# jankammeth/BA-path-planning

Hardware: AMD Instinct MI355X
Metric: SCP iterations/sec (N agents x K waypoints) (higher is better)
Workload: dtype f64

## Files before the change

### ba-path-planning_amd/csrc/scp_common.h

```cpp
#pragma once
#include <hip/hip_runtime.h>

#include <cstdarg>
#include <cstdint>
#include <cstdio>
#include <cstring>

#include "scp_hip.h"

struct scp_stats_mirror {
  scp_pair_stats stats;
  unsigned long long n_spec;
  double pts[6];
  double rel[64];
  volatile unsigned long long seq;
};

constexpr int SCP_SMALL_MAX_WG = 2048;

struct scp_ctx {
  int device;
  int n_cu;
  hipStream_t stream;
  char err[512];
  double* d_scratch;
  double* h_scratch;
  double* h_scratch_dev;
  hipEvent_t ev0, ev1;
  hipEvent_t pair_ev0, pair_ev1;
  bool pair_timed;
  bool pair_ran;
  bool last_pass_small;
  double* tm_scratch;
  size_t tm_bytes;
  uint32_t* cmp_map;
  size_t cmp_map_bytes;
  uint32_t* cmp_tot;
  size_t cmp_tot_bytes;
  scp_stats_mirror* h_mirror;
  scp_stats_mirror* d_mirror;
  unsigned long long mirror_seq;
  unsigned long long* wg_part;
  uint32_t* wg_rows;
  size_t wg_rows_bytes;
  unsigned* d_ticket;
  int timing;
  int small_pass;
  unsigned long long rel_seq;
  void* gen_ws;
  size_t gen_ws_bytes;
  void* sep_ws;
  size_t sep_ws_bytes;
  unsigned long long* sep_n_solved;
  int* h_gen_flag;
  int* d_gen_flag;
};

static inline int scp_fail(scp_ctx* ctx, int code, const char* fmt, ...) {
  if (ctx) {
    va_list ap;
    va_start(ap, fmt);
    vsnprintf(ctx->err, sizeof(ctx->err), fmt, ap);
    va_end(ap);
  }
  return code;
}

#define SCP_HIP_CHECK(ctx, call)                                                                     \
  do {                                                                                               \
    hipError_t e_ = (call);                                                                          \
    if (e_ != hipSuccess)                                                                            \
      return scp_fail((ctx), SCP_ERR_HIP, "%s failed: %s (%s:%d)", #call, hipGetErrorString(e_),    \
                      __FILE__, __LINE__);                                                           \
  } while (0)

#define SCP_REQUIRE(ctx, cond, ...)                                   \
  do {                                                                \
    if (!(cond)) return scp_fail((ctx), SCP_ERR_INVALID, __VA_ARGS__); \
  } while (0)

static inline int64_t scp_pairs(int N) { return (int64_t)N * (N - 1) / 2; }
static inline int scp_cdiv(int64_t a, int64_t b) { return (int)((a + b - 1) / b); }

hipError_t scp_raise_lds_limit(int device, const void* kernel, size_t bytes);

bool scp_wait_host_word(volatile unsigned long long* word, unsigned long long seq, int timeout_s);

int scp_check_pair_range(scp_ctx* ctx, int N, int K, int D, int64_t q_begin, int64_t q_end);

int scp_ctx_wait_stats(scp_ctx* ctx, scp_pair_stats* out);

int scp_violations_from_solution(scp_ctx* ctx, int N, int K, int D, double R, double h, int64_t q_begin, int64_t q_end,
                                 const double* pos_prev, const double* x_tm, const double* p0, const double* v0, double* x_out,
                                 double* pos_out, double feas_tol, int64_t* new_rows, int64_t new_cap, uint32_t* sel_bitmap,
                                 scp_pair_stats* stats, const double* rel_prev ,
                                 int64_t* spec_rows , int64_t spec_cap,
                                 uint32_t* spec_bitmap, double spec_margin, bool* fused);
void scp_ctx_mirror_rel(scp_ctx* ctx, int64_t n, double* out);
int scp_select_from_solution(scp_ctx* ctx, int N, int K, int D, double R, double h, int64_t q_begin, int64_t q_end,
                             const double* x_tm, const double* p0, const double* v0, double* x_out, double* pos_out,
                             double margin, int64_t* sel_rows, int64_t sel_cap, uint32_t* sel_bitmap, scp_pair_stats* stats,
                             bool* fused);
int scp_launch_kinematics_copy(scp_ctx* ctx, int N, int K, int D, double h, const double* acc, const double* p0,
                               const double* v0, double* pos_out, double* vel_out, double* acc_copy);
const double* scp_qp_solution_tm(const scp_qp* qp);

int scp_qp_reset_add_rows_at(scp_qp* qp, const double* x0, int64_t n, const int64_t* rows, const double* pos_prev,
                             const double* p0, const double* v0, double R);
int scp_qp_add_rows_from_pass(scp_qp* qp, int64_t n, const int64_t* rows, const double* eta, const double* l_col,
                              int64_t q_begin, int64_t q_end);

int scp_launch_add_rows_at(scp_ctx* ctx, int N, int K, int D, int64_t base, int64_t n, const int64_t* rows,
                           const double* pos_prev, const double* p0, const double* v0, double R, double h, const double* Qx,
                           int64_t* w_row, int* wk, int* wi, int* wj, double* weta, double* wl, double* zc, double* yc);

int scp_launch_gemm(scp_ctx* ctx, int use_mfma, int R, int M, int C, double alpha, const double* A,
                    const double* X, double beta, double* Y);
int scp_launch_to_time_major(scp_ctx* ctx, int N, int K, int D, const double* src, double* dst);
int scp_launch_from_time_major(scp_ctx* ctx, int N, int K, int D, const double* src, double* dst);
int scp_launch_bounds_time_major(scp_ctx* ctx, int N, int K, int D, double h, const double* limits_host,
                                 const double* space_host, const double* p0, const double* v0,
                                 const double* pf, const double* vf, double* l_tm, double* u_tm,
                                 double* states_out );
```

### ba-path-planning_amd/csrc/scp_kernels.hip

```cpp
#include "scp_common.h"
#include "scp_pair_device.h"

#include <sys/prctl.h>
#include <time.h>

#include <atomic>
#include <chrono>
#include <cmath>
#include <cstdlib>
#include <map>
#include <mutex>
#include <type_traits>
#include <utility>

extern "C" int scp_abi_version(void) { return SCP_ABI_VERSION; }

extern "C" int scp_ctx_create(int device, void* hip_stream, scp_ctx** out) {
  if (!out) return SCP_ERR_INVALID;
  *out = nullptr;
  if (hipSetDevice(device) != hipSuccess) return SCP_ERR_HIP;
  scp_ctx* ctx = new scp_ctx();
  memset(ctx, 0, sizeof(*ctx));
  ctx->device = device;
  ctx->stream = (hipStream_t)hip_stream;
  ctx->timing = 1;
  ctx->small_pass = getenv("SCP_NO_SMALL_PASS") ? 0 : 1;
  if (hipDeviceGetAttribute(&ctx->n_cu, hipDeviceAttributeMultiprocessorCount, device) != hipSuccess) ctx->n_cu = 0;
  if (hipMalloc(&ctx->d_scratch, 72 * sizeof(double)) != hipSuccess ||
      hipMemset(ctx->d_scratch, 0, 72 * sizeof(double)) != hipSuccess ||
      hipHostMalloc(&ctx->h_scratch, 72 * sizeof(double)) != hipSuccess ||
      memset(ctx->h_scratch, 0, 72 * sizeof(double)) == nullptr ||
      hipHostGetDevicePointer((void**)&ctx->h_scratch_dev, ctx->h_scratch, 0) != hipSuccess ||
      hipHostMalloc(&ctx->h_mirror, sizeof(scp_stats_mirror)) != hipSuccess ||
      hipHostGetDevicePointer((void**)&ctx->d_mirror, ctx->h_mirror, 0) != hipSuccess ||
      hipEventCreate(&ctx->ev0) != hipSuccess || hipEventCreate(&ctx->ev1) != hipSuccess ||
      hipEventCreate(&ctx->pair_ev0) != hipSuccess || hipEventCreate(&ctx->pair_ev1) != hipSuccess ||
      hipMalloc(&ctx->wg_part, 4 * SCP_SMALL_MAX_WG * sizeof(unsigned long long)) != hipSuccess ||
      hipMalloc(&ctx->d_ticket, 64) != hipSuccess || hipMemset(ctx->d_ticket, 0, 64) != hipSuccess) {
    delete ctx;
    return SCP_ERR_HIP;
  }
  *out = ctx;
  return SCP_OK;
}

extern "C" int scp_ctx_set_option(scp_ctx* ctx, const char* key, int value) {
  if (!ctx || !key) return SCP_ERR_INVALID;
  if (strcmp(key, "kernel_timing") == 0) {
    ctx->timing = value ? 1 : 0;
    if (!ctx->timing) ctx->pair_timed = false;
    return SCP_OK;
  }
  if (strcmp(key, "single_launch_passes") == 0) {
    ctx->small_pass = value ? 1 : 0;
    return SCP_OK;
  }
  return scp_fail(ctx, SCP_ERR_INVALID, "ctx_set_option: unknown key '%s'", key);
}

extern "C" void scp_ctx_destroy(scp_ctx* ctx) {
  if (!ctx) return;
  (void)hipSetDevice(ctx->device);
  (void)hipStreamSynchronize(ctx->stream);
  (void)hipFree(ctx->d_scratch);
  if (ctx->wg_part) (void)hipFree(ctx->wg_part);
  if (ctx->wg_rows) (void)hipFree(ctx->wg_rows);
  if (ctx->d_ticket) (void)hipFree(ctx->d_ticket);
  if (ctx->cmp_map) (void)hipFree(ctx->cmp_map);
  if (ctx->cmp_tot) (void)hipFree(ctx->cmp_tot);
  if (ctx->tm_scratch) (void)hipFree(ctx->tm_scratch);
  if (ctx->gen_ws) (void)hipFree(ctx->gen_ws);
  if (ctx->sep_ws) (void)hipFree(ctx->sep_ws);
  if (ctx->h_gen_flag) (void)hipHostFree(ctx->h_gen_flag);
  (void)hipHostFree(ctx->h_scratch);
  (void)hipHostFree(ctx->h_mirror);
  (void)hipEventDestroy(ctx->ev0);
  (void)hipEventDestroy(ctx->ev1);
  (void)hipEventDestroy(ctx->pair_ev0);
  (void)hipEventDestroy(ctx->pair_ev1);
  delete ctx;
}

hipError_t scp_raise_lds_limit(int device, const void* kernel, size_t bytes) {
  static std::mutex mu;
  static std::map<std::pair<int, const void*>, size_t> allowed;
  std::lock_guard<std::mutex> lock(mu);
  size_t& have = allowed[std::make_pair(device, kernel)];
  if (have >= bytes) return hipSuccess;
  const hipError_t e = hipFuncSetAttribute(kernel, hipFuncAttributeMaxDynamicSharedMemorySize, (int)bytes);
  if (e == hipSuccess) have = bytes;
  return e;
}

static std::atomic<int> g_host_wait_mode{0};

extern "C" void scp_set_host_wait(int mode) {
  g_host_wait_mode.store(mode == 1 || mode == 2 ? mode : 0, std::memory_order_relaxed);
}

bool scp_wait_host_word(volatile unsigned long long* word, unsigned long long seq, int timeout_s) {
  const auto t0 = std::chrono::steady_clock::now();
  const int wait_mode = g_host_wait_mode.load(std::memory_order_relaxed);
  const bool sleepy = wait_mode != 0;
  const unsigned spin_first = wait_mode == 2 ? 0u : 2000u;
  if (sleepy) {
    static thread_local bool slack_set = false;
    if (!slack_set) {
      (void)prctl(PR_SET_TIMERSLACK, 1000UL, 0UL, 0UL, 0UL);
      slack_set = true;
    }
  }
  unsigned spins = 0;
  while (*word != seq) {
#if defined(__x86_64__) || defined(__i386__)
    __builtin_ia32_pause();
#endif
    ++spins;
    if (sleepy && spins > spin_first) {
      struct timespec ts = {0, 20000};
      nanosleep(&ts, nullptr);
      if ((spins & 0x3FF) == 0 && std::chrono::steady_clock::now() - t0 > std::chrono::seconds(timeout_s)) break;
    } else if ((spins & 0xFFFF) == 0 && std::chrono::steady_clock::now() - t0 > std::chrono::seconds(timeout_s)) {
      break;
    }
  }
  const bool ok = *word == seq;
  __atomic_thread_fence(__ATOMIC_ACQUIRE);
  return ok;
}

int scp_ctx_wait_stats(scp_ctx* ctx, scp_pair_stats* out) {
  if (ctx->mirror_seq == 0) return scp_fail(ctx, SCP_ERR_STATE, "no pass with a row list has run yet");
  if (!scp_wait_host_word(&ctx->h_mirror->seq, ctx->mirror_seq, 30)) {
    SCP_HIP_CHECK(ctx, hipStreamSynchronize(ctx->stream));
    if (ctx->h_mirror->seq != ctx->mirror_seq) return scp_fail(ctx, SCP_ERR_HIP, "pair pass: the stats mirror was not written");
  }
  *out = ctx->h_mirror->stats;
// ... 1945 lines not shown
```

### ba-path-planning_amd/csrc/scp_qp.hip

```cpp
#include "scp_qp_internal.h"
#include "scp_reset_device.h"

#include <chrono>
#include <cmath>
#include <vector>

__device__ inline double sum_partials(const double* part) {
  double s = 0.0;
  for (int b = 0; b < NPART; ++b) s += part[b];
  return s;
}

__global__ __launch_bounds__(256) void dot_partial_kernel(int64_t n, const double* __restrict__ a,
                                                           const double* __restrict__ b, double* __restrict__ part) {
  __shared__ double s[4];
  double acc = 0.0;
  for (int64_t t = (int64_t)blockIdx.x * 256 + threadIdx.x; t < n; t += (int64_t)NPART * 256) acc += a[t] * b[t];
#pragma unroll
  for (int o = 32; o > 0; o >>= 1) acc += __shfl_xor(acc, o);
  if ((threadIdx.x & 63) == 0) s[threadIdx.x >> 6] = acc;
  __syncthreads();
  if (threadIdx.x == 0) part[blockIdx.x] = (s[0] + s[1]) + (s[2] + s[3]);
}

// ... 1082 lines not shown
  SCP_REQUIRE(ctx, dst->N == src->N && dst->K == src->K && dst->D == src->D && dst->h == src->h,
              "qp_clone_state: shapes differ");
  if (!src->reset_done) return scp_fail(ctx, SCP_ERR_STATE, "qp_clone_state: source has no state");
  if (src->nW > dst->row_cap)
    return scp_fail(ctx, SCP_ERR_CAPACITY, "qp_clone_state: %lld rows exceed the capacity %lld", (long long)src->nW,
                    (long long)dst->row_cap);
  hipStream_t s = ctx->stream;
  const size_t nf = (size_t)src->Rf * src->C * sizeof(double), nx = (size_t)src->K * src->C * sizeof(double);
  const size_t nw = (size_t)src->nW;
  const QpDev &a = src->d, &b = dst->d;
#define CP(field, bytes) SCP_HIP_CHECK(ctx, hipMemcpyAsync(b.field, a.field, (bytes), hipMemcpyDeviceToDevice, s))
  CP(lf, nf); CP(uf, nf); CP(zf, nf); CP(yf, nf); CP(x, nx);
  CP(states, (size_t)4 * src->C * sizeof(double));
  if (nw) {
    CP(w_row, nw * sizeof(int64_t)); CP(w_k, nw * sizeof(int)); CP(w_i, nw * sizeof(int)); CP(w_j, nw * sizeof(int));
    CP(w_eta, nw * src->D * sizeof(double)); CP(w_l, nw * sizeof(double)); CP(zc, nw * sizeof(double));
    CP(yc, nw * sizeof(double));
  }
#undef CP
  memcpy(dst->lim, src->lim, sizeof(dst->lim));
  memcpy(dst->space, src->space, sizeof(dst->space));
  dst->steps_since_reset = src->steps_since_reset;
  dst->nW = src->nW;
  dst->persist_cap_nW = -1;
  dst->rho = src->rho;
  dst->st = src->st;
  dst->problem_set = true;
  qp_on_x_set(dst, false);
  QP_CHECK(build_kkt(dst));
  dst->reset_done = true;
  SCP_HIP_CHECK(ctx, hipStreamSynchronize(s));
  return SCP_OK;
}

extern "C" int scp_qp_get_solution(scp_qp* qp, double* x_out) {
  if (!qp) return SCP_ERR_INVALID;
  SCP_REQUIRE(qp->ctx, x_out, "qp_get_solution: null pointer");
  if (!qp->reset_done) return scp_fail(qp->ctx, SCP_ERR_STATE, "qp_get_solution: no solve yet");
  return scp_launch_from_time_major(qp->ctx, qp->N, qp->K, qp->D, qp->d.x, x_out);
}

const double* scp_qp_solution_tm(const scp_qp* qp) { return qp->d.x; }

extern "C" int scp_qp_get_duals(scp_qp* qp, double* y_fixed, double* y_col) {
  if (!qp) return SCP_ERR_INVALID;
  scp_ctx* ctx = qp->ctx;
  if (!qp->reset_done) return scp_fail(ctx, SCP_ERR_STATE, "qp_get_duals: no solve yet");
  const int N = qp->N, K = qp->K, D = qp->D;
  const int64_t C = qp->C;
  if (y_fixed) {
    QP_CHECK(scp_launch_from_time_major(ctx, N, K - 1, D, qp->d.yf, y_fixed));
    int64_t src = (int64_t)(K - 1) * C, dst = (int64_t)N * (K - 1) * D;
    for (int b = 0; b < 3; ++b) {
      QP_CHECK(scp_launch_from_time_major(ctx, N, K, D, qp->d.yf + src, y_fixed + dst));
      src += (int64_t)K * C;
      dst += (int64_t)N * K * D;
    }
  }
  if (y_col && qp->nW > 0)
    SCP_HIP_CHECK(ctx, hipMemcpyAsync(y_col, qp->d.yc, qp->nW * sizeof(double), hipMemcpyDeviceToDevice, ctx->stream));
  return SCP_OK;
}

extern "C" int scp_qp_peek(scp_qp* qp, const char* name, double* out, int64_t cap, int64_t* n_out) {
  if (!qp) return SCP_ERR_INVALID;
  scp_ctx* ctx = qp->ctx;
  SCP_REQUIRE(ctx, name && out && n_out, "qp_peek: null pointer");
  const QpDev& d = qp->d;
  const int64_t nf = (int64_t)qp->Rf * qp->C, nx = (int64_t)qp->K * qp->C;
  const double* src = nullptr;
  int64_t n = 0;
  if (!strcmp(name, "fx")) { src = d.fx; n = nf; }
  else if (!strcmp(name, "qx")) { src = scp_qp_qx(qp); n = nx; }
  else if (!strcmp(name, "gval")) { src = d.gval; n = 2 * qp->nW; }
  else if (!strcmp(name, "zf")) { src = d.zf; n = nf; }
  else if (!strcmp(name, "yf")) { src = d.yf; n = nf; }
  else if (!strcmp(name, "zc")) { src = d.zc; n = qp->nW; }
  else if (!strcmp(name, "yc")) { src = d.yc; n = qp->nW; }
  else if (!strcmp(name, "x")) { src = d.x; n = nx; }
  else if (!strcmp(name, "w_eta")) { src = d.w_eta; n = qp->nW * qp->D; }
  else if (!strcmp(name, "w_l")) { src = d.w_l; n = qp->nW; }
  else if (!strcmp(name, "p")) { src = d.p; n = nx; }
  else if (!strcmp(name, "qp")) { src = d.s0p; n = nx; }
  else return scp_fail(ctx, SCP_ERR_INVALID, "qp_peek: unknown array %s", name);
  *n_out = n;
  if (n > cap) return scp_fail(ctx, SCP_ERR_CAPACITY, "qp_peek: %lld doubles needed", (long long)n);
  if (n > 0) SCP_HIP_CHECK(ctx, hipMemcpyAsync(out, src, (size_t)n * sizeof(double), hipMemcpyDeviceToDevice, ctx->stream));
  return SCP_OK;
}

extern "C" int scp_qp_debug_set(scp_qp* qp, const char* key, int value) {
  if (!qp || !key) return SCP_ERR_INVALID;
  if (!strcmp(key, "persist_fault")) {
    if (value >= 0) qp->persist_fault = value;
    return qp->persist_fault;
  }
  if (!strcmp(key, "persist_off")) {
    if (value >= 0) qp->persist_off = value != 0;
    return qp->persist_off ? 1 : 0;
  }
  if (!strcmp(key, "persist_gave_up_total")) return qp->persist_gave_up_total;
  return scp_fail(qp->ctx, SCP_ERR_INVALID, "qp_debug_set: unknown key %s", key);
}
```

### ba-path-planning_amd/csrc/scp_qp_fused.hip

```cpp
#include "scp_qp_device.h"
#include "scp_pair_device.h"
#include "scp_reset_device.h"
#include <cstdlib>

namespace {

using namespace scpdev;
constexpr int FT = 1024;
constexpr int NWV = FT / 64;

#ifdef SCP_PHASE_PROFILE
__device__ unsigned long long scp_phase_clk[64];
#define PHASE_MARK(slot)                                                                      \
  do {                                                                                        \
    if (blockIdx.x == gridDim.x / 2 && threadIdx.x == 0) scp_phase_clk[slot] = wall_clock64(); \
  } while (0)
#else
#define PHASE_MARK(slot) ((void)0)
#endif

constexpr int SQ_BLOCKS = 128;
template <int E>
__global__ __launch_bounds__(FT) void cg1_col_kernel(int K, int Rf, int64_t C, double rho, double h,
                                                      const double* __restrict__ pMinv, const double* __restrict__ wrow,
// ... 578 lines not shown
    tc += e[d] * (fma(a, pi[d], qi[d]) - fma(a, pj[d], qj[d]));
    ax += e[d] * (fma(aa, pi[d], qi[d]) - fma(aa, pj[d], qj[d]));
  }
  const double zh = alpha * tc + (1.0 - alpha) * z;
  const double zn = fmax(zh + y / rho_c, lo);
  const double yn = y + rho_c * (zh - zn);
  yc[n] = yn;
  zc[n] = zn;
  if (dyc) dyc[n] = fmin(yn - y, 0.0);
  const double g = (rho_c * zn - yn) - rho_c * ax;
  gval[posi] = g;
  gval[posj] = g;
}

template <int D, bool INIT>
__global__ __launch_bounds__(256) void rows_value_kernel(int64_t nW, int64_t C, double rho, const int* __restrict__ wk,
                                                          const int* __restrict__ wi, const int* __restrict__ wj,
                                                          const double* __restrict__ weta, const double* __restrict__ Q,
                                                          const double* __restrict__ zc, const double* __restrict__ yc,
                                                          const int* __restrict__ pos_i, const int* __restrict__ pos_j,
                                                          double* __restrict__ gval) {
  const int64_t n = (int64_t)blockIdx.x * 256 + threadIdx.x;
  if (n >= nW) return;
  const int64_t bi = (int64_t)wk[n] * C + (int64_t)wi[n] * D;
  const int64_t bj = (int64_t)wk[n] * C + (int64_t)wj[n] * D;
  double ax = 0.0;
#pragma unroll
  for (int d = 0; d < D; ++d) ax += weta[n * D + d] * (Q[bi + d] - Q[bj + d]);
  const double g = INIT ? (rho * zc[n] - yc[n]) - rho * ax : rho * ax;
  gval[pos_i[n]] = g;
  gval[pos_j[n]] = g;
}

#define FUSED_LAUNCHED(qp) SCP_HIP_CHECK((qp)->ctx, hipGetLastError())

template <typename Kern>
int allow_lds(scp_qp* qp, Kern kernel, size_t bytes) {
  if (bytes <= 64 * 1024) return SCP_OK;
  SCP_HIP_CHECK(qp->ctx, scp_raise_lds_limit(qp->ctx->device, reinterpret_cast<const void*>(kernel), bytes));
  return SCP_OK;
}

}

int scp_qp_qp0_iterations(scp_qp* qp, int nit, double* dy_out) {
  const QpDev& d = qp->d;
  hipStream_t s = qp->ctx->stream;
  const int K = qp->K, Rf = qp->Rf;
  const int64_t C = qp->C;
  const int nblk = (int)((C + CB - 1) / CB);
  const size_t lds = (size_t)CB * (pad_col(Rf) + 3 * pad_col(K)) * sizeof(double);
  if (K <= 64) {
    int rc = allow_lds(qp, qp0_col_kernel<1>, lds);
    if (rc) return rc;
    hipLaunchKernelGGL(qp0_col_kernel<1>, dim3(nblk), dim3(FT), lds, s, K, Rf, C, qp->rho, qp->st.sigma, qp->st.alpha, qp->h,
                       nit, d.pMinv, d.wrow, d.lf, d.uf, d.x, d.zf, d.yf, dy_out);
  } else {
    int rc = allow_lds(qp, qp0_col_kernel<2>, lds);
    if (rc) return rc;
    hipLaunchKernelGGL(qp0_col_kernel<2>, dim3(nblk), dim3(FT), lds, s, K, Rf, C, qp->rho, qp->st.sigma, qp->st.alpha, qp->h,
                       nit, d.pMinv, d.wrow, d.lf, d.uf, d.x, d.zf, d.yf, dy_out);
  }
  FUSED_LAUNCHED(qp);
  return SCP_OK;
}

namespace {
constexpr int CSR1_MAX_CELLS = 16384;
constexpr int64_t CSR1_MAX_ROWS = 1 << 18;
struct CsrNewRows {
  int64_t n, base;
  const int64_t* rows;
  const double *pos_prev, *p0, *v0;
  double R, h;
  int N;
  int64_t* w_row;
  double* wl;
};
__global__ void csr_small_kernel(int64_t nW, int K, int ncell, int D, int64_t C, double rho, int* __restrict__ wk,
                                 int* __restrict__ wi, int* __restrict__ wj, double* __restrict__ weta,
                                 const double* __restrict__ Qx, double* __restrict__ zc, double* __restrict__ yc,
                                 int* __restrict__ ptr, int* __restrict__ ent, double* __restrict__ coef,
                                 int* __restrict__ pos_i, int* __restrict__ pos_j, double* __restrict__ gval, CsrNewRows nr);
}

int scp_qp_cg1_prepare(scp_qp* qp) {
  if (qp->dv.carried) return SCP_OK;
  const QpDev& d = qp->d;
  hipStream_t s = qp->ctx->stream;
  const int K = qp->K;
  const int64_t C = qp->C;
  const double rho_c = qp->rho * qp->st.rho_col_scale;
  QP_CHECK(scp_qp_exact_qx(qp, true));
  const double* Qx = scp_qp_qx(qp);
  if (qp->dv.vals_rho_c == rho_c) {
  } else if (!qp->dv.lists && qp->nW > 0 && qp->nW <= CSR1_MAX_ROWS && qp->N * K <= CSR1_MAX_CELLS) {
    const int ncell = qp->N * K;
    hipLaunchKernelGGL(csr_small_kernel, dim3(1), dim3(1024), (size_t)ncell * sizeof(int), s, qp->nW, K, ncell, qp->D, C, rho_c,
                       d.w_k, d.w_i, d.w_j, d.w_eta, Qx, d.zc, d.yc, d.cell_ptr, d.ent_code, d.coef, d.pos_i, d.pos_j, d.gval,
                       CsrNewRows{});
    FUSED_LAUNCHED(qp);
  } else {
    QP_CHECK(scp_qp_csr_ensure(qp));
    const dim3 rgrid((unsigned)((qp->nW + 255) / 256)), rblock(256);
    if (qp->D == 2)
      hipLaunchKernelGGL((rows_value_kernel<2, true>), rgrid, rblock, 0, s, qp->nW, C, rho_c, d.w_k, d.w_i, d.w_j, d.w_eta, Qx,
                         d.zc, d.yc, d.pos_i, d.pos_j, d.gval);
    else
      hipLaunchKernelGGL((rows_value_kernel<3, true>), rgrid, rblock, 0, s, qp->nW, C, rho_c, d.w_k, d.w_i, d.w_j, d.w_eta, Qx,
                         d.zc, d.yc, d.pos_i, d.pos_j, d.gval);
    FUSED_LAUNCHED(qp);
  }
  qp_on_cg1_prepared(qp);
  return SCP_OK;
}

int scp_qp_install_rows_small(scp_qp* qp, int64_t n, const int64_t* rows, const double* pos_prev, const double* p0,
                              const double* v0, double R, const double* Qx, bool* done) {
  *done = false;
  const QpDev& d = qp->d;
  const int K = qp->K;
  const int64_t nW = qp->nW + n;
  if (!qp->dv.qx || n <= 0 || nW > CSR1_MAX_ROWS || qp->N * K > CSR1_MAX_CELLS) return SCP_OK;
  const int ncell = qp->N * K;
  const double rho_c = qp->rho * qp->st.rho_col_scale;
  CsrNewRows nr{n, qp->nW, rows, pos_prev, p0, v0, R, qp->h, qp->N, d.w_row, d.w_l};
  hipLaunchKernelGGL(csr_small_kernel, dim3(1), dim3(1024), (size_t)ncell * sizeof(int), qp->ctx->stream, nW, K, ncell, qp->D,
                     qp->C, rho_c, d.w_k, d.w_i, d.w_j, d.w_eta, Qx, d.zc, d.yc, d.cell_ptr, d.ent_code, d.coef, d.pos_i,
                     d.pos_j, d.gval, nr);
  FUSED_LAUNCHED(qp);
  *done = true;
  return SCP_OK;
}

int scp_qp_cg1_iteration(scp_qp* qp, int* cg_count, bool emit_dy) {
  const QpDev& d = qp->d;
  double* dyf = emit_dy ? d.dyf : nullptr;
  double* dyc = emit_dy ? d.dyc : nullptr;
  hipStream_t s = qp->ctx->stream;
  const int K = qp->K, Rf = qp->Rf;
  const int64_t C = qp->C;
  const int nblk = (int)((C + CB - 1) / CB);
  double* Qp = d.s0p;
  double* Fp = d.tf;
  double* part_rz = d.part;
  double* part_sq = d.part + SCP_PART_CAP / 2;
  const double rho_c = qp->rho * qp->st.rho_col_scale;
  QP_CHECK(scp_qp_cg1_prepare(qp));
  double* Qx = scp_qp_qx(qp);
  double* Qn = scp_qp_qx(qp, true);
  const size_t lds = (size_t)CB * (pad_col(Rf) + 5 * pad_col(K)) * sizeof(double);
  int npart = nblk;
  if (K > SCP_FUSED_MAX_K) {
    npart = (int)C;
    hipLaunchKernelGGL(cg1_colK_kernel, dim3((unsigned)C), dim3((unsigned)((K + 63) / 64 * 64)), (size_t)2 * K * sizeof(double), s, K, Rf,
                       C, qp->rho, qp->h, d.Minv, d.wrow, d.x, d.fx, d.zf, d.yf, qp->N, qp->D, d.cell_ptr, d.coef, d.gval, d.p,
                       Qp, Fp, part_rz);
  } else if (K <= 64) {
    int rc = allow_lds(qp, cg1_col_kernel<1>, lds);
    if (rc) return rc;
    hipLaunchKernelGGL(cg1_col_kernel<1>, dim3(nblk), dim3(FT), lds, s, K, Rf, C, qp->rho, qp->h, d.pMinv, d.wrow, d.x, d.fx,
                       d.zf, d.yf, qp->N, qp->D, d.cell_ptr, d.coef, d.gval, d.p, Qp, Fp, part_rz);
  } else {
    int rc = allow_lds(qp, cg1_col_kernel<2>, lds);
    if (rc) return rc;
    hipLaunchKernelGGL(cg1_col_kernel<2>, dim3(nblk), dim3(FT), lds, s, K, Rf, C, qp->rho, qp->h, d.pMinv, d.wrow, d.x, d.fx,
                       d.zf, d.yf, qp->N, qp->D, d.cell_ptr, d.coef, d.gval, d.p, Qp, Fp, part_rz);
  }
  FUSED_LAUNCHED(qp);
  const dim3 rblock(256);
  const int inline_sq = qp->nW <= SQ_INLINE_MAX ? 1 : 0;
  if (!inline_sq) {
    if (qp->D == 2)
      hipLaunchKernelGGL(cg1_rows_sq_kernel<2>, dim3(SQ_BLOCKS), rblock, 0, s, qp->nW, C, rho_c, d.w_k, d.w_i, d.w_j,
                         d.w_eta, Qp, part_sq);
    else
      hipLaunchKernelGGL(cg1_rows_sq_kernel<3>, dim3(SQ_BLOCKS), rblock, 0, s, qp->nW, C, rho_c, d.w_k, d.w_i, d.w_j,
                         d.w_eta, Qp, part_sq);
    FUSED_LAUNCHED(qp);
  }
  const int nblk8 = (nblk + 7) & ~7;
  const int eblocks = nblk8 * ((Rf + K + 16 * UPD_RPT - 1) / (16 * UPD_RPT));
  const dim3 ugrid((unsigned)(eblocks + (qp->nW + 255) / 256));
  if (qp->D == 2)
// ... 138 lines not shown
  for (int64_t n = tid; n < nW; n += 1024) {
    atomicAdd(&csr_cnt[cell_of(wk[n], wi[n], K)], 1);
    atomicAdd(&csr_cnt[cell_of(wk[n], wj[n], K)], 1);
  }
  __syncthreads();
  {
    int v[SC], tot = 0;
#pragma unroll
    for (int e = 0; e < SC; ++e) {
      v[e] = SC * tid + e < ncell ? csr_cnt[SC * tid + e] : 0;
      tot += v[e];
    }
    int incl = tot;
#pragma unroll
    for (int o = 1; o < 64; o <<= 1) {
      const int t = __shfl_up(incl, o);
      if (lane >= o) incl += t;
    }
    if (lane == 63) wsum[wave] = incl;
    __syncthreads();
    int run = incl - tot;
    for (int w = 0; w < wave; ++w) run += wsum[w];
#pragma unroll
    for (int e = 0; e < SC; ++e) {
      if (SC * tid + e < ncell) {
        csr_cnt[SC * tid + e] = run;
        ptr[SC * tid + e] = run;
      }
      run += v[e];
    }
    if (tid == 1023) ptr[ncell] = run;
  }
  __syncthreads();
  for (int64_t n = tid; n < nW; n += 1024) {
    ent[atomicAdd(&csr_cnt[cell_of(wk[n], wi[n], K)], 1)] = (int)(2 * n);
    ent[atomicAdd(&csr_cnt[cell_of(wk[n], wj[n], K)], 1)] = (int)(2 * n + 1);
  }
  __syncthreads();
  for (int c = tid; c < ncell; c += 1024) {
    const int b = c ? csr_cnt[c - 1] : 0, e = csr_cnt[c];
    for (int i = b + 1; i < e; ++i) {
      const int v = ent[i];
      int j = i - 1;
      while (j >= b && ent[j] > v) {
        ent[j + 1] = ent[j];
        --j;
      }
      ent[j + 1] = v;
    }
  }
  __syncthreads();
  for (int64_t t = tid; t < 2 * nW; t += 1024) {
    const int code = ent[t];
    const int n = code >> 1, side = code & 1;
    for (int d = 0; d < D; ++d) coef[t * D + d] = side ? -weta[(int64_t)n * D + d] : weta[(int64_t)n * D + d];
    if (side) pos_j[n] = (int)t;
    else pos_i[n] = (int)t;
  }
  __syncthreads();
  for (int64_t n = tid; n < nW; n += 1024) {
    const int64_t bi = (int64_t)wk[n] * C + (int64_t)wi[n] * D;
    const int64_t bj = (int64_t)wk[n] * C + (int64_t)wj[n] * D;
    double ax = 0.0;
    for (int d = 0; d < D; ++d)
      ax += weta[n * D + d] * (COH ? load_coherent(Qx + bi + d) - load_coherent(Qx + bj + d) : Qx[bi + d] - Qx[bj + d]);
    const double g = (rho * zc[n] - yc[n]) - rho * ax;
    gval[pos_i[n]] = g;
    gval[pos_j[n]] = g;
  }
}

__global__ __launch_bounds__(1024) void csr_small_kernel(int64_t nW, int K, int ncell, int D, int64_t C, double rho,
                                                          int* __restrict__ wk, int* __restrict__ wi,
                                                          int* __restrict__ wj, double* __restrict__ weta,
                                                          const double* __restrict__ Qx, double* __restrict__ zc,
                                                          double* __restrict__ yc, int* __restrict__ ptr,
                                                          int* __restrict__ ent, double* __restrict__ coef,
                                                          int* __restrict__ pos_i, int* __restrict__ pos_j,
                                                          double* __restrict__ gval, CsrNewRows nr) {
  extern __shared__ int csr_cnt[];
  csr_small_body<false>(csr_cnt, nW, K, ncell, D, C, rho, wk, wi, wj, weta, Qx, zc, yc, ptr, ent, coef, pos_i, pos_j, gval, nr);
}

struct ResetArgs {
  int N, Rf;
  const double *x0, *F, *S0;
  double *x, *zf, *fx, *yf;
};
__global__ __launch_bounds__(1024) void reset_install_kernel(ResetArgs ra, int64_t nW, int K, int ncell, int D, int64_t C,
                                                              double rho, int* __restrict__ wk, int* __restrict__ wi,
                                                              int* __restrict__ wj, double* __restrict__ weta,
                                                              double* __restrict__ Qx, double* __restrict__ zc,
                                                              double* __restrict__ yc, int* __restrict__ ptr,
                                                              int* __restrict__ ent, double* __restrict__ coef,
                                                              int* __restrict__ pos_i, int* __restrict__ pos_j,
                                                              double* __restrict__ gval, CsrNewRows nr,
                                                              unsigned* __restrict__ ticket) {
  extern __shared__ __attribute__((aligned(16))) char ri_lds[];
  __shared__ int last_sh;
  qp_reset_body<true>(threadIdx.x, threadIdx.x < 256, reinterpret_cast<double*>(ri_lds), ra.N, K, D, ra.Rf, ra.x0, ra.F, ra.S0,
                      ra.x, ra.zf, ra.fx, Qx, ra.yf);
  wait_stores_performed();
  __syncthreads();
  if (threadIdx.x == 0) last_sh = atomicAdd(ticket, 1u) == gridDim.x - 1 ? 1 : 0;
  __syncthreads();
  if (!last_sh) return;
  if (threadIdx.x == 0) *ticket = 0u;
  csr_small_body<true>(reinterpret_cast<int*>(ri_lds), nW, K, ncell, D, C, rho, wk, wi, wj, weta, Qx, zc, yc, ptr, ent, coef,
                       pos_i, pos_j, gval, nr);
}

}

int scp_qp_reset_install_small(scp_qp* qp, const double* x0, int64_t n, const int64_t* rows, const double* pos_prev,
                               const double* p0, const double* v0, double R, double* Qx, bool* done) {
  *done = false;
  const QpDev& d = qp->d;
  const int K = qp->K;
  if (n <= 0 || n > CSR1_MAX_ROWS || qp->N * K > CSR1_MAX_CELLS) return SCP_OK;
  const int ncell = qp->N * K;
  const double rho_c = qp->rho * qp->st.rho_col_scale;
  const size_t lds = std::max((size_t)K * RESET_COLS * sizeof(double), (size_t)ncell * sizeof(int));
  CsrNewRows nr{n, 0, rows, pos_prev, p0, v0, R, qp->h, qp->N, d.w_row, d.w_l};
  ResetArgs ra{qp->N, qp->Rf, x0, d.F, d.S0, d.x, d.zf, d.fx, d.yf};
  hipLaunchKernelGGL(reset_install_kernel, dim3((unsigned)scp_cdiv(qp->C, RESET_COLS)), dim3(1024), lds, qp->ctx->stream, ra, n,
                     K, ncell, qp->D, qp->C, rho_c, d.w_k, d.w_i, d.w_j, d.w_eta, Qx, d.zc, d.yc, d.cell_ptr, d.ent_code,
                     d.coef, d.pos_i, d.pos_j, d.gval, nr, qp->ctx->d_ticket + 2);
  FUSED_LAUNCHED(qp);
  *done = true;
  return SCP_OK;
}

namespace {
__global__ __launch_bounds__(256) void csr_rowval_kernel(int64_t nW, int mode, double rho, const double* __restrict__ zc,
                                                          const double* __restrict__ yc, const double* __restrict__ vec,
                                                          const int* __restrict__ pos_i, const int* __restrict__ pos_j,
                                                          double* __restrict__ gval, const double* __restrict__ vec2,
                                                          double* __restrict__ gval2) {
  const int64_t n = (int64_t)blockIdx.x * 256 + threadIdx.x;
  if (n >= nW) return;
  if (gval2) {
    const double g2 = vec2[n];
    gval2[pos_i[n]] = g2;
    gval2[pos_j[n]] = g2;
  }
  const double g = mode == 0 ? rho * zc[n] - yc[n] : (mode == 1 ? yc[n] : vec[n]);
  gval[pos_i[n]] = g;
  gval[pos_j[n]] = g;
}

__global__ __launch_bounds__(256) void csr_gather_kernel(int K, int N, int D, const int* __restrict__ ptr,
                                                          const double* __restrict__ coef,
                                                          const double* __restrict__ gval, double* __restrict__ G) {
  const int64_t t = (int64_t)blockIdx.x * 256 + threadIdx.x;
  const int64_t C = (int64_t)N * D;
  if (t >= C * K) return;
  const int k = (int)(t / C), col = (int)(t % C);
  const int agent = col / D, d = col - agent * D;
  const int cell = cell_of(k, agent, K);
  double acc = 0.0;
  const int t1 = ptr[cell + 1];
  for (int e = ptr[cell]; e < t1; ++e) acc += coef[(size_t)e * D + d] * gval[e];
  G[t] = acc;
}

}

int scp_qp_csr_ensure(scp_qp* qp) {
  if (qp->dv.lists) return SCP_OK;
  const QpDev& d = qp->d;
  hipStream_t s = qp->ctx->stream;
  const int ncell = qp->N * qp->K;
  SCP_REQUIRE(qp->ctx, 2 * qp->nW < 0x3FFFFFFF, "csr_build: too many working rows for 32-bit entry codes");
  SCP_HIP_CHECK(qp->ctx, hipMemsetAsync(d.cell_ptr, 0, (size_t)(ncell + 1) * sizeof(int), s));
  if (qp->nW > 0) {
    const dim3 rgrid((unsigned)((qp->nW + 255) / 256));
    hipLaunchKernelGGL(csr_count_kernel, rgrid, dim3(256), 0, s, qp->nW, qp->K, d.w_k, d.w_i, d.w_j, d.cell_ptr);
    const int sblk = (ncell + SCAN_CELLS - 1) / SCAN_CELLS;
    hipLaunchKernelGGL(csr_scan_local_kernel, dim3(sblk), dim3(256), 0, s, ncell, d.cell_ptr, d.scan_tot);
    hipLaunchKernelGGL(csr_scan_add_kernel, dim3(sblk), dim3(256), 0, s, ncell, sblk, d.cell_ptr, d.cell_cur, d.scan_tot);
    hipLaunchKernelGGL(csr_fill_kernel, rgrid, dim3(256), 0, s, qp->nW, qp->K, d.w_k, d.w_i, d.w_j, d.cell_cur, d.ent_code);
    hipLaunchKernelGGL(csr_sort_kernel, dim3((ncell + 255) / 256), dim3(256), 0, s, ncell, d.cell_ptr, d.ent_code);
    hipLaunchKernelGGL(csr_finish_kernel, dim3((unsigned)((2 * qp->nW + 255) / 256)), dim3(256), 0, s, 2 * qp->nW, qp->D,
                       d.ent_code, d.w_eta, d.coef, d.pos_i, d.pos_j);
    FUSED_LAUNCHED(qp);
  }
  qp_on_lists_built(qp);
  return SCP_OK;
}

int scp_qp_csr_scatter(scp_qp* qp, int mode, const double* vec) {
  QP_CHECK(scp_qp_csr_ensure(qp));
  const QpDev& d = qp->d;
  hipStream_t s = qp->ctx->stream;
  const int64_t nx = (int64_t)qp->K * qp->C;
  hipLaunchKernelGGL(csr_rowval_kernel, dim3((unsigned)((qp->nW + 255) / 256)), dim3(256), 0, s, qp->nW, mode,
                     qp->rho * qp->st.rho_col_scale, d.zc, d.yc, vec, d.pos_i, d.pos_j, d.gval, (const double*)nullptr, (double*)nullptr);
  hipLaunchKernelGGL(csr_gather_kernel, dim3((unsigned)((nx + 255) / 256)), dim3(256), 0, s, qp->K, qp->N, qp->D,
                     d.cell_ptr, d.coef, d.gval, d.G);
  FUSED_LAUNCHED(qp);
  return SCP_OK;
}

int scp_qp_rows_gather(scp_qp* qp, const double* Q) {
  const QpDev& d = qp->d;
  hipStream_t s = qp->ctx->stream;
  QP_CHECK(scp_qp_csr_ensure(qp));
  const int64_t C = qp->C, nx = (int64_t)qp->K * C;
  const double rho_c = qp->rho * qp->st.rho_col_scale;
  const dim3 rgrid((unsigned)((qp->nW + 255) / 256)), rblock(256);
  if (qp->D == 2)
    hipLaunchKernelGGL((rows_value_kernel<2, false>), rgrid, rblock, 0, s, qp->nW, C, rho_c, d.w_k, d.w_i, d.w_j, d.w_eta, Q,
                       d.zc, d.yc, d.pos_i, d.pos_j, d.gval);
  else
    hipLaunchKernelGGL((rows_value_kernel<3, false>), rgrid, rblock, 0, s, qp->nW, C, rho_c, d.w_k, d.w_i, d.w_j, d.w_eta, Q,
                       d.zc, d.yc, d.pos_i, d.pos_j, d.gval);
  hipLaunchKernelGGL(csr_gather_kernel, dim3((unsigned)((nx + 255) / 256)), dim3(256), 0, s, qp->K, qp->N, qp->D,
                     d.cell_ptr, d.coef, d.gval, d.G);
  FUSED_LAUNCHED(qp);
  return SCP_OK;
}

namespace {
struct PackDesc {
  const double* src;
  double* dst;
  int R, M;
};
struct PackArgs {
  PackDesc m[2];
};
__global__ __launch_bounds__(256) void pack_operands_kernel(PackArgs a) {
  const PackDesc d = a.m[blockIdx.y];
  const int nks = (d.M + 3) >> 2;
  const int64_t total = (int64_t)((d.R + 15) >> 4) * nks * 64;
  for (int64_t e = (int64_t)blockIdx.x * 256 + threadIdx.x; e < total; e += (int64_t)gridDim.x * 256) {
    const int lane = (int)(e & 63);
    const int64_t q = e >> 6;
    const int ks = (int)(q % nks), t = (int)(q / nks);
    const int row = t * 16 + (lane & 15), k = 4 * ks + (lane >> 4);
    d.dst[e] = (row < d.R && k < d.M) ? d.src[(size_t)row * d.M + k] : 0.0;
  }
}
}

int scp_qp_pack_operands(scp_qp* qp) {
  const QpDev& d = qp->d;
  const int K = qp->K;
  PackArgs a;
  a.m[0] = {d.Minv, d.pMinv, K, K};
  a.m[1] = {d.T, d.pT, K, K};
  hipLaunchKernelGGL(pack_operands_kernel, dim3(16, 2), dim3(256), 0, qp->ctx->stream, a);
// ... 310 lines not shown
```

Measured before the change: 413.6.

## Build CSR cell lists for large problems in a single fused kernel launch

Adds a csr_large_kernel in which each workgroup owns a contiguous range of cells and, inside one launch, counts entries, scans, fills, insertion-sorts and writes coefficients and optional row values. This replaces the six-kernel count/scan/add/fill/sort/finish sequence when the problem exceeds the small path. Every workgroup scans all working rows, so redundant global reads grow with the grid size. The change aims to cut launch overhead and intermediate global traffic. It also adds debug peek access to the integer CSR arrays and an option to disable the new path.

```diff
diff --git a/ba-path-planning_amd/csrc/scp_common.h b/ba-path-planning_amd/csrc/scp_common.h
--- a/ba-path-planning_amd/csrc/scp_common.h
+++ b/ba-path-planning_amd/csrc/scp_common.h
@@ -46,6 +46,7 @@
   unsigned* d_ticket;
   int timing;
   int small_pass;
+  int large_launch;
   unsigned long long rel_seq;
   void* gen_ws;
   size_t gen_ws_bytes;
diff --git a/ba-path-planning_amd/csrc/scp_kernels.hip b/ba-path-planning_amd/csrc/scp_kernels.hip
--- a/ba-path-planning_amd/csrc/scp_kernels.hip
+++ b/ba-path-planning_amd/csrc/scp_kernels.hip
@@ -25,6 +25,7 @@
   ctx->stream = (hipStream_t)hip_stream;
   ctx->timing = 1;
   ctx->small_pass = getenv("SCP_NO_SMALL_PASS") ? 0 : 1;
+  ctx->large_launch = 1;
   if (hipDeviceGetAttribute(&ctx->n_cu, hipDeviceAttributeMultiprocessorCount, device) != hipSuccess) ctx->n_cu = 0;
   if (hipMalloc(&ctx->d_scratch, 72 * sizeof(double)) != hipSuccess ||
       hipMemset(ctx->d_scratch, 0, 72 * sizeof(double)) != hipSuccess ||
@@ -53,6 +54,10 @@
   }
   if (strcmp(key, "single_launch_passes") == 0) {
     ctx->small_pass = value ? 1 : 0;
+    return SCP_OK;
+  }
+  if (strcmp(key, "single_launch_large") == 0) {
+    ctx->large_launch = value ? 1 : 0;
     return SCP_OK;
   }
   return scp_fail(ctx, SCP_ERR_INVALID, "ctx_set_option: unknown key '%s'", key);
diff --git a/ba-path-planning_amd/csrc/scp_qp.hip b/ba-path-planning_amd/csrc/scp_qp.hip
--- a/ba-path-planning_amd/csrc/scp_qp.hip
+++ b/ba-path-planning_amd/csrc/scp_qp.hip
@@ -1188,9 +1188,22 @@
   else if (!strcmp(name, "w_l")) { src = d.w_l; n = qp->nW; }
   else if (!strcmp(name, "p")) { src = d.p; n = nx; }
   else if (!strcmp(name, "qp")) { src = d.s0p; n = nx; }
+  else if (!strcmp(name, "coef")) { src = d.coef; n = 2 * qp->nW * qp->D; }
+  const void* isrc = nullptr;
+  int64_t ni = 0;
+  if (src) {}
+  else if (!strcmp(name, "cell_ptr")) { isrc = d.cell_ptr; ni = (int64_t)qp->N * qp->K + 1; }
+  else if (!strcmp(name, "ent_code")) { isrc = d.ent_code; ni = 2 * qp->nW; }
+  else if (!strcmp(name, "pos_i")) { isrc = d.pos_i; ni = qp->nW; }
+  else if (!strcmp(name, "pos_j")) { isrc = d.pos_j; ni = qp->nW; }
   else return scp_fail(ctx, SCP_ERR_INVALID, "qp_peek: unknown array %s", name);
+  if (isrc) n = (ni + 1) / 2;
   *n_out = n;
   if (n > cap) return scp_fail(ctx, SCP_ERR_CAPACITY, "qp_peek: %lld doubles needed", (long long)n);
+  if (isrc) {
+    if (ni > 0) SCP_HIP_CHECK(ctx, hipMemcpyAsync(out, isrc, (size_t)ni * sizeof(int), hipMemcpyDeviceToDevice, ctx->stream));
+    return SCP_OK;
+  }
   if (n > 0) SCP_HIP_CHECK(ctx, hipMemcpyAsync(out, src, (size_t)n * sizeof(double), hipMemcpyDeviceToDevice, ctx->stream));
   return SCP_OK;
 }
diff --git a/ba-path-planning_amd/csrc/scp_qp_fused.hip b/ba-path-planning_amd/csrc/scp_qp_fused.hip
--- a/ba-path-planning_amd/csrc/scp_qp_fused.hip
+++ b/ba-path-planning_amd/csrc/scp_qp_fused.hip
@@ -684,6 +684,8 @@
                                  const double* __restrict__ Qx, double* __restrict__ zc, double* __restrict__ yc,
                                  int* __restrict__ ptr, int* __restrict__ ent, double* __restrict__ coef,
                                  int* __restrict__ pos_i, int* __restrict__ pos_j, double* __restrict__ gval, CsrNewRows nr);
+bool csr_large_ok(const scp_qp* qp);
+int csr_large_build(scp_qp* qp, bool with_vals, double rho_c, const double* Qx);
 }
 
 int scp_qp_cg1_prepare(scp_qp* qp) {
@@ -702,6 +704,8 @@
                        d.w_k, d.w_i, d.w_j, d.w_eta, Qx, d.zc, d.yc, d.cell_ptr, d.ent_code, d.coef, d.pos_i, d.pos_j, d.gval,
                        CsrNewRows{});
     FUSED_LAUNCHED(qp);
+  } else if (!qp->dv.lists && csr_large_ok(qp)) {
+    QP_CHECK(csr_large_build(qp, true, rho_c, Qx));
   } else {
     QP_CHECK(scp_qp_csr_ensure(qp));
     const dim3 rgrid((unsigned)((qp->nW + 255) / 256)), rblock(256);
@@ -1006,6 +1010,139 @@
   csr_small_body<false>(csr_cnt, nW, K, ncell, D, C, rho, wk, wi, wj, weta, Qx, zc, yc, ptr, ent, coef, pos_i, pos_j, gval, nr);
 }
 
+template <int D>
+__device__ inline double row_value_init(int64_t n, int64_t C, double rho, const int* __restrict__ wk, const int* __restrict__ wi,
+                                        const int* __restrict__ wj, const double* __restrict__ weta,
+                                        const double* __restrict__ Q, const double* __restrict__ zc,
+                                        const double* __restrict__ yc) {
+  const int64_t bi = (int64_t)wk[n] * C + (int64_t)wi[n] * D;
+  const int64_t bj = (int64_t)wk[n] * C + (int64_t)wj[n] * D;
+  double ax = 0.0;
+#pragma unroll
+  for (int d = 0; d < D; ++d) ax += weta[n * D + d] * (Q[bi + d] - Q[bj + d]);
+  return (rho * zc[n] - yc[n]) - rho * ax;
+}
+
+constexpr int CSRL_THREADS = 1024;
+constexpr int CSRL_MAX_CPW = 8192;
+template <int D>
+__global__ __launch_bounds__(CSRL_THREADS) void csr_large_kernel(int64_t nW, int K, int ncell, int cpw, int64_t C, double rho,
+                                                                  int with_vals, const int* __restrict__ wk,
+                                                                  const int* __restrict__ wi, const int* __restrict__ wj,
+                                                                  const double* __restrict__ weta,
+                                                                  const double* __restrict__ Qx, const double* __restrict__ zc,
+                                                                  const double* __restrict__ yc, int* __restrict__ ptr,
+                                                                  int* __restrict__ ent, double* __restrict__ coef,
+                                                                  int* __restrict__ pos_i, int* __restrict__ pos_j,
+                                                                  double* __restrict__ gval) {
+  extern __shared__ int csrl_cnt[];
+  __shared__ int wsum[CSRL_THREADS / 64], wbelow[CSRL_THREADS / 64];
+  const int tid = threadIdx.x, lane = tid & 63, wave = tid >> 6;
+  const int c0 = (int)blockIdx.x * cpw;
+  const int nc = min(cpw, ncell - c0);
+  for (int c = tid; c < nc; c += CSRL_THREADS) csrl_cnt[c] = 0;
+  __syncthreads();
+  int below = 0;
+  for (int64_t n = tid; n < nW; n += CSRL_THREADS) {
+    const int k = wk[n];
+    const int ci = cell_of(k, wi[n], K) - c0, cj = cell_of(k, wj[n], K) - c0;
+    if (ci < 0) ++below;
+    else if (ci < nc) atomicAdd(&csrl_cnt[ci], 1);
+    if (cj < 0) ++below;
+    else if (cj < nc) atomicAdd(&csrl_cnt[cj], 1);
+  }
+#pragma unroll
+  for (int o = 32; o > 0; o >>= 1) below += __shfl_xor(below, o);
+  if (lane == 0) wbelow[wave] = below;
+  __syncthreads();
+  const int sc = cpw / CSRL_THREADS;
+  int tot = 0;
+  for (int e = 0; e < sc; ++e)
+    if (sc * tid + e < nc) tot += csrl_cnt[sc * tid + e];
+  int incl = tot;
+#pragma unroll
+  for (int o = 1; o < 64; o <<= 1) {
+    const int t = __shfl_up(incl, o);
+    if (lane >= o) incl += t;
+  }
+  if (lane == 63) wsum[wave] = incl;
+  __syncthreads();
+  int base = 0;
+  for (int w = 0; w < CSRL_THREADS / 64; ++w) base += wbelow[w];
+  int run = base + incl - tot;
+  for (int w = 0; w < wave; ++w) run += wsum[w];
+  for (int e = 0; e < sc; ++e) {
+    const int c = sc * tid + e;
+    if (c < nc) {
+      const int v = csrl_cnt[c];
+      csrl_cnt[c] = run;
+      ptr[c0 + c] = run;
+      run += v;
+    }
+  }
+  if (tid == CSRL_THREADS - 1 && c0 + nc == ncell) ptr[ncell] = run;
+  __syncthreads();
+  for (int64_t n = tid; n < nW; n += CSRL_THREADS) {
+    const int k = wk[n];
+    const int ci = cell_of(k, wi[n], K) - c0, cj = cell_of(k, wj[n], K) - c0;
+    if (ci >= 0 && ci < nc) ent[atomicAdd(&csrl_cnt[ci], 1)] = (int)(2 * n);
+    if (cj >= 0 && cj < nc) ent[atomicAdd(&csrl_cnt[cj], 1)] = (int)(2 * n + 1);
+  }
+  __syncthreads();
+  for (int c = tid; c < nc; c += CSRL_THREADS) {
+    const int b = c ? csrl_cnt[c - 1] : base, e = csrl_cnt[c];
+    for (int i = b + 1; i < e; ++i) {
+      const int v = ent[i];
+      int j = i - 1;
+      while (j >= b && ent[j] > v) {
+        ent[j + 1] = ent[j];
+        --j;
+      }
+      ent[j + 1] = v;
+    }
+  }
+  __syncthreads();
+  const int end = csrl_cnt[nc - 1];
+  for (int t = base + tid; t < end; t += CSRL_THREADS) {
+    const int code = ent[t];
+    const int n = code >> 1, side = code & 1;
+#pragma unroll
+    for (int d = 0; d < D; ++d) coef[(int64_t)t * D + d] = side ? -weta[(int64_t)n * D + d] : weta[(int64_t)n * D + d];
+    if (side) pos_j[n] = t;
+    else pos_i[n] = t;
+    if (with_vals) gval[t] = row_value_init<D>(n, C, rho, wk, wi, wj, weta, Qx, zc, yc);
+  }
+}
+
+inline int csr_large_cpw(int ncell) {
+  const int cpw = (int)scp_cdiv(scp_cdiv(ncell, 128), CSRL_THREADS) * CSRL_THREADS;
+  return std::min(cpw, CSRL_MAX_CPW);
+}
+
+bool csr_large_ok(const scp_qp* qp) {
+  return qp->ctx->large_launch && qp->nW > 0 && (int64_t)qp->N * qp->K <= (int64_t)CSRL_MAX_CPW * 65535;
+}
+
+int csr_large_build(scp_qp* qp, bool with_vals, double rho_c, const double* Qx) {
+  const QpDev& d = qp->d;
+  const int ncell = qp->N * qp->K;
+  SCP_REQUIRE(qp->ctx, 2 * qp->nW < 0x3FFFFFFF, "csr_build: too many working rows for 32-bit entry codes");
+  const int cpw = csr_large_cpw(ncell);
+  const dim3 grid((unsigned)scp_cdiv(ncell, cpw)), block(CSRL_THREADS);
+  const size_t lds = (size_t)cpw * sizeof(int);
+  if (qp->D == 2)
+    hipLaunchKernelGGL(csr_large_kernel<2>, grid, block, lds, qp->ctx->stream, qp->nW, qp->K, ncell, cpw, qp->C, rho_c,
+                       with_vals ? 1 : 0, d.w_k, d.w_i, d.w_j, d.w_eta, Qx, d.zc, d.yc, d.cell_ptr, d.ent_code, d.coef, d.pos_i,
+                       d.pos_j, d.gval);
+  else
+    hipLaunchKernelGGL(csr_large_kernel<3>, grid, block, lds, qp->ctx->stream, qp->nW, qp->K, ncell, cpw, qp->C, rho_c,
+                       with_vals ? 1 : 0, d.w_k, d.w_i, d.w_j, d.w_eta, Qx, d.zc, d.yc, d.cell_ptr, d.ent_code, d.coef, d.pos_i,
+                       d.pos_j, d.gval);
+  FUSED_LAUNCHED(qp);
+  qp_on_lists_built(qp);
+  return SCP_OK;
+}
+
 struct ResetArgs {
   int N, Rf;
   const double *x0, *F, *S0;
@@ -1092,6 +1229,7 @@
 
 int scp_qp_csr_ensure(scp_qp* qp) {
   if (qp->dv.lists) return SCP_OK;
+  if (csr_large_ok(qp)) return csr_large_build(qp, false, 0.0, nullptr);
   const QpDev& d = qp->d;
   hipStream_t s = qp->ctx->stream;
   const int ncell = qp->N * qp->K;
```

After: 420.8, median of 6. No clear change (+1.7%).
